# spaceandtimefdn/blitzar

Hardware: AMD Instinct MI355X
Metric: MSM throughput (scalar-point ops/sec) (higher is better)
Workload: dtype u32; 1 GPU; curve25519_msm_n2^20_252bit; columns_per_gpu=1, rows=1048576, parallelism=columns x1

## Files before the change

### __graft_entry__.py

```python
import os
import subprocess
import sys

ROOT = os.path.dirname(os.path.abspath(__file__))
if ROOT not in sys.path:
    sys.path.insert(0, ROOT)


def build():
    from blitzar_amd import build as bz_build
    bz_build.build()
    hooks_dir = os.path.join(ROOT, "tests", "native", "_build")
    os.makedirs(hooks_dir, exist_ok=True)
    hooks = os.path.join(hooks_dir, "libbz_hooks.so")
    src = os.path.join(ROOT, "tests", "native", "hooks.cpp")
    if not os.path.exists(hooks) or os.path.getmtime(hooks) < os.path.getmtime(src):
        subprocess.run(["g++", "-O2", "-std=c++20", "-fPIC", "-shared", "-I" + ROOT, src, "-o", hooks],
                       check=True)
    src = os.path.join(ROOT, "tests", "native", "tile_digest_check.cc")
    newest = max(os.path.getmtime(src),
                 os.path.getmtime(os.path.join(ROOT, "blitzar_amd", "csrc", "msm", "tile_digest.h")))
    for exe, flags in (("tile_digest_check", ["-O2"]),
                       ("tile_digest_check_san", ["-O1", "-g", "-fsanitize=address,undefined",
                                                  "-fno-sanitize-recover=all"])):
        exe = os.path.join(hooks_dir, exe)
        if not os.path.exists(exe) or os.path.getmtime(exe) < newest:
            subprocess.run(["g++", *flags, "-std=c++20", "-I" + ROOT, src, "-o", exe], check=True)
    pb_dir = os.path.join(ROOT, "tools", "pipeline_bench")
    lib_so = os.path.join(ROOT, "blitzar_amd", "lib", "libblitzar_amd.so")
    os.makedirs(os.path.join(pb_dir, "_build"), exist_ok=True)
    for tool in ("pipeline_bench", "multi_device_check", "hostapi_bench", "caller_table_bench"):
        exe = os.path.join(pb_dir, "_build", tool)
        src = os.path.join(pb_dir, tool + ".cc")
        if (not os.path.exists(exe)
                or os.path.getmtime(exe) < max(os.path.getmtime(src), os.path.getmtime(lib_so))):
            subprocess.run(["/opt/rocm/bin/hipcc", "-O2", "-std=c++17",
                            "-I" + os.path.join(ROOT, "include"), "-I" + pb_dir, src,
                            "-L" + os.path.dirname(lib_so), "-lblitzar_amd",
                            "-Wl,-rpath,$ORIGIN/../../../blitzar_amd/lib", "-o", exe], check=True)
    mc_src = os.path.join(ROOT, "tools", "multi_commitment", "benchmark.cc")
    mc_exe = os.path.join(ROOT, "tools", "multi_commitment", "_build", "multi_commitment")
    os.makedirs(os.path.dirname(mc_exe), exist_ok=True)
    if (not os.path.exists(mc_exe)
            or os.path.getmtime(mc_exe) < max(os.path.getmtime(mc_src), os.path.getmtime(lib_so))):
        subprocess.run(["g++", "-O2", "-std=c++17", "-I" + os.path.join(ROOT, "include"), mc_src,
                        "-L" + os.path.dirname(lib_so), "-lblitzar_amd",
                        "-Wl,-rpath,$ORIGIN/../../../blitzar_amd/lib", "-Wl,-rpath,/opt/rocm/lib",
                        "-o", mc_exe], check=True)
    exe = os.path.join(hooks_dir, "sig_ours")
    src = os.path.join(ROOT, "tests", "native", "boundary", "signatures.cc")
    if (not os.path.exists(exe)
            or os.path.getmtime(exe) < max(os.path.getmtime(src), os.path.getmtime(lib_so))):
        subprocess.run(["g++", "-O1", "-std=c++17", "-I" + os.path.join(ROOT, "include"),
                        '-DBZ_API_HEADER="blitzar_api.h"', src, "-L" + os.path.dirname(lib_so),
                        "-lblitzar_amd", "-Wl,-rpath,$ORIGIN/../../../blitzar_amd/lib",
                        "-Wl,-rpath,/opt/rocm/lib", "-o", exe], check=True)
    mt_dir = os.path.join(ROOT, "tools", "mt19937")
    mt_so = os.path.join(mt_dir, "_build", "libmtstream.so")
    mt_src = os.path.join(mt_dir, "mtstream.cc")
    os.makedirs(os.path.dirname(mt_so), exist_ok=True)
    if not os.path.exists(mt_so) or os.path.getmtime(mt_so) < os.path.getmtime(mt_src):
        subprocess.run(["g++", "-O2", "-std=c++17", "-fPIC", "-shared", "-pthread", mt_src, "-o",
                        mt_so], check=True)
    subprocess.run([sys.executable, os.path.join(ROOT, "oracle", "ref", "build_ref.py")], check=True)
    from tests import device_hooks
    device_hooks.build()
    import blitzar_amd.api as api
    api.load()


def smoke():
    import numpy as np
    from blitzar_amd import api
    from oracle import ref_oracle
    lib = api.load()
    assert lib.bzamd_device_count() > 0, "smoke() needs a GPU"
    api.reset_for_testing()
# ... 28 lines not shown
```

### blitzar_amd/csrc/msm/curve_traits.h

```cpp
#pragma once

#include "blitzar_amd/csrc/curve/ed25519.h"
#include "blitzar_amd/csrc/curve/ed29.h"
#include "blitzar_amd/csrc/curve/ed16_wave.h"
#include "blitzar_amd/csrc/curve/sw29.h"
#include "blitzar_amd/csrc/curve/sw29_coop.h"
#include "blitzar_amd/csrc/curve/sw_wave.h"
#include "blitzar_amd/csrc/curve/weierstrass.h"

namespace bz {

template <int N> struct sw_api_affine {
  u64 X[N];
  u64 Y[N];
  u8 infinity;
};
static_assert(sizeof(sw_api_affine<4>) == 72);
static_assert(sizeof(sw_api_affine<6>) == 104);

struct ed25519_msm {
  static constexpr unsigned curve_id = 0;
  using point = ed29_point;
  using addend = ed29_cached_packed;
  using api_projective = ed_point;
// ... 8 lines not shown
  static constexpr double call_table_entry_cost = 1.0;

  BZ_HD static point identity() { return ed29::identity(); }
  BZ_HD static point add(const point& a, const point& b) { return ed29::add(a, b); }
  BZ_HD static point dbl_n(const point& a, int k) { return ed29::dbl_n(a, k); }
  BZ_HD static point neg(const point& a) { return ed29::neg(a); }
  BZ_HD static void accumulate(point& acc, const addend& q, bool negate) {
    acc = ed29::add_cached(acc, ed29::unpack(q), negate);
  }
  using operand = ed29_cached;
  BZ_HD static operand stage(const addend& q) {
    operand o = ed29::unpack(q);
    f29::pin(o.YpX);
    f29::pin(o.YmX);
    f29::pin(o.Z);
    f29::pin(o.T2d);
    return o;
  }
  BZ_HD static void accumulate(point& acc, const operand& q, bool negate) {
    acc = ed29::add_cached(acc, q, negate);
  }
  static constexpr bool has_signed_gather = true;
  BZ_HD static addend gather(const addend* table, u32 row, bool negate) {
    return ed29::gather_signed(table, row, negate);
  }
  BZ_HD static void accumulate_gathered(point& acc, const operand& q, bool negate) {
    acc = ed29::add_cached_presigned(acc, q, negate);
  }
  static constexpr bool first_pinned = true;
  BZ_HD static point first_gathered(const operand& q, bool negate) {
    return ed29::from_cached_presigned(q, negate);
  }
  BZ_HD static addend make_addend(const void* api_generators, u64 i) {
    return ed29::pack(ed29::cached_from_ed(static_cast<const ed_point*>(api_generators)[i]));
  }
  BZ_HD static addend addend_from_api_projective(const void* projective, u64 i) {
    return make_addend(projective, i);
  }
  BZ_HD static void encode(u8* out, const point& p) { ristretto29::encode(out, p); }
  BZ_HD static void store_projective(u8* out, const point& p) {
    *reinterpret_cast<ed_point*>(out) = ed29::to_ed(p);
  }
  BZ_HD static point point_from_api_projective(const void* projective, u64 i) {
    return ed29::from_ed(static_cast<const ed_point*>(projective)[i]);
  }
  BZ_HD static void store_api_generator(u8* out, const point& p) { store_projective(out, p); }
  BZ_HD static point point_from_api_generator(const void* api_generators, u64 i) {
    return point_from_api_projective(api_generators, i);
  }
  static constexpr u32 batch_points_per_lane = 4;
  using batch_fe = fe29;
  BZ_HD static fe29 batch_one() { return f29::one(); }
  BZ_HD static fe29 batch_mul(const fe29& a, const fe29& b) { return f29::mul(a, b); }
  BZ_HD static fe29 batch_z(const point& p, bool& is_identity) {
    is_identity = false;
    return p.Z;
  }
  static constexpr size_t compact_size = 120;
  BZ_HD static void store_compact(u8* out, const point& p, const fe29& zinv, bool) {
    const fe29 x = f29::mul(p.X, zinv), y = f29::mul(p.Y, zinv);
    const fe51 c[3] = {f29::to_fe51(x), f29::to_fe51(y), f29::to_fe51(f29::mul(x, y))};
    u64* o = reinterpret_cast<u64*>(out);
    for (int k = 0; k < 3; ++k)
      for (int i = 0; i < 5; ++i) o[5 * k + i] = c[k].v[i];
  }
#if defined(__HIPCC__)
  __device__ static fe29 batch_wave_invert(const fe29& z) {
    const ed16w::lane_ctx c = ed16w::make_ctx(ed16w::wave_scratch());
    const fe29 t = ed16w::pow22523(c, z);
    return f29::mul(f29::sqn(t, 3), f29::mul(f29::sq(z), z));
  }
#endif
  static constexpr bool has_wave_horner = true;
#if defined(__HIPCC__)
  __device__ static point wave_horner(const point& acc, bool have_acc, point* window_sums,
                                      u32 stride, u32 num_windows, u32 window_bits) {
    const ed16w::lane_ctx c = ed16w::make_ctx(ed16w::wave_scratch());
    for (u32 w = c.lane; w < num_windows; w += 64) {
      point* slot = window_sums + static_cast<size_t>(w) * stride;
      const ed29_cached_packed q = ed29::pack(ed29::to_cached(*slot));
      *reinterpret_cast<ed29_cached_packed*>(slot) = q;
    }
    ed16w::wave_lds_sync();
    u32 state = ed16w::identity(c);
    if (have_acc) state = ed16w::load_point(c, acc);
    for (u32 i = num_windows; i-- > 0;) {
      if (have_acc || i + 1 != num_windows) {
        for (u32 k = 0; k < window_bits; ++k) state = ed16w::dbl(c, state);
      }
      const u32* q = reinterpret_cast<const u32*>(window_sums + static_cast<size_t>(i) * stride);
      state = ed16w::add_cached(c, state, ed16w::load_words(c, q));
    }
    return ed16w::store_point(c, state);
  }
  __device__ static void wave_chain(point* out, u64 stride, const point& g, u32 windows, u32 bits) {
    const ed16w::lane_ctx c = ed16w::make_ctx(ed16w::wave_scratch());
    u32 state = ed16w::load_point(c, g);
#pragma unroll 1
    for (u32 w = 0;; ++w) {
      const point p = ed16w::store_point(c, state);
      if (c.lane == 0) out[static_cast<u64>(w) * stride] = p;
      if (w + 1 >= windows) break;
#pragma unroll 1
      for (u32 k = 0; k < bits; ++k) state = ed16w::dbl(c, state);
    }
  }
  static constexpr bool has_wave_add_multiple = true;
  static constexpr bool reduce_scan_few_columns_only = false;
  __device__ static point wave_add_multiple(const point& v, const point& s, u32 m) {
    __shared__ ed29_cached_packed addend[2];
    const ed16w::lane_ctx c = ed16w::make_ctx(ed16w::wave_scratch());
    if (c.lane < 2) addend[c.lane] = ed29::pack(ed29::to_cached(c.lane == 0 ? s : v));
    ed16w::wave_lds_sync();
    const u32 sq = ed16w::load_words(c, addend[0].w), vq = ed16w::load_words(c, addend[1].w);
    u32 state = ed16w::identity(c);
    for (int bit = 31 - __builtin_clz(m); bit >= 0; --bit) {
      state = ed16w::dbl(c, state);
      if ((m >> bit) & 1) state = ed16w::add_cached(c, state, sq);
    }
    state = ed16w::add_cached(c, state, vq);
    return ed16w::store_point(c, state);
  }
  static constexpr bool has_wave_encode = true;
  static constexpr bool has_coop_add = false;
  __device__ static void wave_encode(u8* out, const point& p) {
    const ed16w::lane_ctx c = ed16w::make_ctx(ed16w::wave_scratch());
    u64 w[4];
    ristretto29::encode_words(w, p, [&c](const fe29& z) { return ed16w::pow22523(c, z); });
    if (c.lane == 0) {
      for (int i = 0; i < 4; ++i)
        for (int j = 0; j < 8; ++j) out[8 * i + j] = static_cast<u8>(w[i] >> (8 * j));
    }
  }
#endif
};

struct ed25519_niels_msm : ed25519_msm {
  using addend = ed29_niels;
  static constexpr int accumulate_launch_waves = accumulate_waves_per_simd;
  BZ_HD static void accumulate(point& acc, const addend& q, bool negate) {
    acc = ed29::add_niels(acc, q, negate);
  }
  BZ_HD static point first(const addend& q, bool negate) { return ed29::from_niels(q, negate); }
  static constexpr bool has_signed_gather = false;
  static constexpr double call_table_entry_cost = 0.88;
  using operand = ed29_niels;
  BZ_HD static operand stage(const addend& q) {
    operand o = q;
    f29::pin(o.YpX);
    f29::pin(o.YmX);
    f29::pin(o.T2d);
    return o;
  }
  BZ_HD static addend make_addend(const void* api_generators, u64 i) {
    return ed29::to_niels(ed29::from_ed(static_cast<const ed_point*>(api_generators)[i]));
  }
  BZ_HD static addend addend_from_api_projective(const void* projective, u64 i) {
    return make_addend(projective, i);
  }
  static constexpr bool has_batched_prepare = true;
  BZ_HD static fe29 batch_load_z(const void* api_generators, u64 i) {
    return f29::from_fe51(static_cast<const ed_point*>(api_generators)[i].Z);
  }
  BZ_HD static addend batch_make_addend(const void* api_generators, u64 i, const fe29& zinv) {
    const ed_point& g = static_cast<const ed_point*>(api_generators)[i];
    return niels_of(f29::from_fe51(g.X), f29::from_fe51(g.Y), zinv);
  }
  BZ_HD static addend addend_from_point(const point& p, const fe29& zinv, bool) {
    return niels_of(p.X, p.Y, zinv);
  }
  BZ_HD static addend niels_of(const fe29& big_x, const fe29& big_y, const fe29& zinv) {
    const fe29 x = f29::mul(big_x, zinv);
    const fe29 y = f29::mul(big_y, zinv);
    ed29_niels n;
    n.YpX = f29::weak_reduce(f29::add(y, x));
    n.YmX = f29::weak_reduce(f29::sub(y, x));
    n.T2d = f29::mul(f29::mul(x, y), f29::const_2d());
    for (int k = 0; k < 5; ++k) n.pad[k] = 0;
    return n;
  }
};

template <class G29, unsigned CurveId> struct sw_msm_base {
  static constexpr unsigned curve_id = CurveId;
  static constexpr double call_table_entry_cost = 1.0;
  using G64 = typename G29::G64;
  using F64 = typename G64::F;
  static constexpr int N64 = F64::N;
  using point = typename G29::point;
  using addend = typename G29::packed;
  using api_projective = typename G64::point;
  using api_affine = sw_api_affine<N64>;
  static constexpr size_t api_generator_size = sizeof(api_affine);
  static constexpr size_t projective_size = sizeof(api_projective);
  static constexpr int accumulate_waves_per_simd = G29::N <= 9 ? 3 : 2;
  static constexpr int accumulate_launch_waves = accumulate_waves_per_simd;
  static constexpr bool accumulate_pinned = G29::N <= 9;
  static constexpr bool has_batched_prepare = false;
  static constexpr bool has_signed_gather = false;
  static constexpr bool has_wave_encode = false;
  static constexpr bool has_wave_add_multiple = true;
  static constexpr bool reduce_scan_few_columns_only = true;
#if defined(__HIPCC__)
  __device__ static point wave_add_multiple(const point& v, const point& s, u32 m) {
    using W = sww::wave<G29>;
    const typename W::ctx c = W::make_ctx(sww::wave_scratch());
    const u32 sq = W::load_point_value(c, s), vq = W::load_point_value(c, v);
    u32 st = sq;
    for (int bit = 30 - __builtin_clz(m); bit >= 0; --bit) {
      st = W::dbl(c, st);
      if ((m >> bit) & 1) st = W::add(c, st, sq);
    }
    return W::store_point(c, W::add(c, st, vq));
  }
#endif
  static constexpr bool has_wave_horner = true;
// ... 149 lines not shown
```

### blitzar_amd/csrc/msm/curve_tu.h

```cpp
#pragma once

#include "blitzar_amd/csrc/msm/dispatch.h"
#include "blitzar_amd/csrc/msm/engine.h"
#include "blitzar_amd/csrc/fixed/partition_table.h"
#include "blitzar_amd/csrc/fixed/partition_table_device.h"
#include "blitzar_amd/csrc/msm/host_backend.h"

namespace bz {

template <class C>
__global__ void __launch_bounds__(256)
    k_prepare_addends_projective(typename C::addend* __restrict__ addends,
                                 const typename C::api_projective* __restrict__ points, u64 n) {
  const u64 i = static_cast<u64>(blockIdx.x) * blockDim.x + threadIdx.x;
  if (i >= n) return;
  addends[i] = C::addend_from_api_projective(points, i);
}

template <class C, bool Encode = true>
__global__ void __launch_bounds__(64)
    k_fold_encode(u8* __restrict__ out, const typename C::api_projective* __restrict__ partials,
                  u32 num_partials, u32 num_outputs) {
  const u32 k = blockIdx.x * blockDim.x + threadIdx.x;
  if (k >= num_outputs) return;
// ... 158 lines not shown
    launch_prepare_addends<R>(static_cast<typename R::addend*>(d_addends), d_api_generators, n,
                              stream);
    BZ_HIP_CHECK(hipGetLastError());
  }
  static void prepare_resident_projective(void* d_addends, const void* d_projective, u64 n,
                                          hipStream_t stream) {
    if (n == 0) return;
    hipLaunchKernelGGL((k_prepare_addends_projective<R>), dim3(ceil_div_u32(n, 256)), dim3(256), 0,
                       stream, static_cast<typename R::addend*>(d_addends),
                       static_cast<const typename R::api_projective*>(d_projective), n);
    BZ_HIP_CHECK(hipGetLastError());
  }
  static const typename R::addend* build_call_table(msm_context& ctx, const void* d_api_generators,
                                                    u64 n, const window_table& t,
                                                    hipStream_t stream) {
    using point = typename R::point;
    using addend = typename R::addend;
    const u64 rows = t.stride * t.windows;
    ctx.call_table.reset(device_arena::padded(sizeof(addend) * (rows + 1)) +
                             device_arena::padded(sizeof(point) * (rows + 1)),
                         stream);
    addend* table = ctx.call_table.take<addend>(rows + 1);
    point* points = ctx.call_table.take<point>(rows + 1);
    hipStream_t bs = stream;
    if (ctx.table_overlap) {
      ctx.make_side_stream();
      ctx.table_fork.record(stream);
      ctx.table_fork.wait(ctx.side);
      bs = ctx.side;
    }
    if (t.stride <= wave_chain_max_rows<R>() && ctx.wave_chain) {
      hipLaunchKernelGGL((k_chain_points_wave<R>), dim3(static_cast<u32>(t.stride)), dim3(64), 0, bs,
                         points, d_api_generators, n, t.stride, t.windows, t.bits);
    } else {
      hipLaunchKernelGGL((k_chain_points<R>), dim3(ceil_div_u32(t.stride, 64)), dim3(64), 0, bs,
                         points, d_api_generators, n, t.stride, t.windows, static_cast<int>(t.bits));
    }
    hipLaunchKernelGGL((k_points_to_addends<R>),
                       dim3(ceil_div_u32(rows, 256ull * R::batch_points_per_lane)), dim3(256), 0, bs,
                       table, points, rows);
    BZ_HIP_CHECK(hipGetLastError());
    g_kernel_launches += 2;
    ctx.call_tables_built += 1;
    ctx.call_table_rows = table;
    if (ctx.table_overlap) {
      ctx.table_ready.record(bs);
      ctx.table_pending = true;
    }
    return table;
  }
  static const typename R::addend* call_table_locked(msm_context& ctx,
                                                     const std::vector<host_column>& cols,
                                                     const void* d_api_generators,
                                                     window_table& shape, hipStream_t stream) {
    shape = window_table{};
    shape.windows = 0;
    if (!ctx.call_tables || d_api_generators == nullptr) return nullptr;
    const call_table_choice ch =
        choose_call_table(cols, ctx.tuning, sizeof(typename R::addend), R::call_table_entry_cost,
                          ctx.force_call_table_bits);
    if (ch.shape.windows == 0) return nullptr;
    const u64 n = generator_rows_of(cols);
    shape = ch.shape;
    return build_call_table(ctx, d_api_generators, n, shape, stream);
  }
  static const void* call_table(msm_context& ctx, const std::vector<host_column>& cols,
                                const void* d_api_generators, window_table* shape,
                                hipStream_t stream) {
    std::lock_guard<std::recursive_mutex> lock(ctx.mu);
    ctx.order_after_previous(stream);
    const void* table = call_table_locked(ctx, cols, d_api_generators, *shape, stream);
    if (table != nullptr) ctx.mark_enqueued(stream);
    return table;
  }
  static void msm(msm_context& ctx, u8* d_out, u32 out_stride, bool projective_out,
                  const std::vector<host_column>& cols, const void* d_addends,
                  const void* d_api_generators, hipStream_t stream, bool generators_keyed) {
    if (cols.empty()) return;
    std::lock_guard<std::recursive_mutex> lock(ctx.mu);
    configure_sort_kernels(ctx);
    ctx.order_after_previous(stream);
    if (d_addends == nullptr) {
      window_table shape;
      const typename R::addend* table = call_table_locked(ctx, cols, d_api_generators, shape, stream);
      if (table != nullptr) {
        msm_enqueue_locked<R>(ctx, d_out, out_stride, projective_out, cols, table, nullptr, stream,
                              &shape, ctx.force_call_table_bits != 0);
        return;
      }
    }
    msm_enqueue_locked<C>(ctx, d_out, out_stride, projective_out, cols,
                          static_cast<const typename C::addend*>(d_addends), d_api_generators, stream,
                          nullptr, false, generators_keyed);
  }
  static void prepare_addends(void* d_addends, const void* d_api_generators, u64 n,
                              hipStream_t stream) {
    launch_prepare_addends<C>(static_cast<typename C::addend*>(d_addends), d_api_generators, n,
                              stream);
    BZ_HIP_CHECK(hipGetLastError());
  }
  static void prepare_addends_projective(void* d_addends, const void* d_projective, u64 n,
                                         hipStream_t stream) {
    if (n == 0) return;
    hipLaunchKernelGGL((k_prepare_addends_projective<C>), dim3(ceil_div_u32(n, 256)), dim3(256), 0,
                       stream, static_cast<typename C::addend*>(d_addends),
                       static_cast<const typename C::api_projective*>(d_projective), n);
    BZ_HIP_CHECK(hipGetLastError());
  }
  static void msm_host_entry(u8* out, u32 out_stride, bool projective_out,
                             const std::vector<host_column>& cols, const void* generators,
                             bool generators_projective, u64 num_generators) {
    std::vector<typename H::addend> addends(num_generators);
    for (u64 i = 0; i < num_generators; ++i) {
      addends[i] = generators_projective
                       ? H::addend_from_api_projective(generators, i)
                       : H::make_addend(generators, i);
    }
    msm_host<H>(out, out_stride, projective_out, cols, addends.data());
  }
  static void fold_encode_host(u8* out, const void* partials, u32 num_partials, u32 num_outputs) {
    for (u32 k = 0; k < num_outputs; ++k) {
      typename C::point acc = C::identity();
      for (u32 r = 0; r < num_partials; ++r) {
        acc = C::add(acc,
                     C::point_from_api_projective(partials, static_cast<u64>(r) * num_outputs + k));
      }
      C::encode(out + static_cast<u64>(k) * C::output_size, acc);
    }
  }
  static void fold_shifted_host(u8* out, const void* pieces, const u32* piece_counts,
                                u32 num_outputs, u32 shift_bits) {
    u64 first = 0;
    for (u32 k = 0; k < num_outputs; ++k) {
      typename C::point acc = C::identity();
      for (u32 j = piece_counts[k]; j-- > 0;) {
        if (j + 1 != piece_counts[k]) acc = C::dbl_n(acc, static_cast<int>(shift_bits));
        acc = C::add(acc, C::point_from_api_projective(pieces, first + j));
      }
      C::store_projective(out + static_cast<u64>(k) * C::projective_size, acc);
      first += piece_counts[k];
// ... 59 lines not shown
```

### blitzar_amd/csrc/msm/engine.h

```cpp
#pragma once

#include <cstdlib>
#include <cstring>
#include <mutex>
#include <type_traits>
#include <vector>

#include "blitzar_amd/csrc/base/device.h"
#include "blitzar_amd/csrc/msm/kernels.h"

namespace bz {

constexpr int kNumStages = 6;
struct stage_timer {
  struct span {
    int stage;
    hipEvent_t begin, end;
  };
  bool enabled = false;
  std::vector<span> spans;
  size_t calls = 0;
  size_t capacity_calls = 0;

  unsigned stage_mask = 0x3f;
// ... 51 lines not shown
};

struct stage_mark {
  hipEvent_t ev = nullptr;
  hipStream_t on = nullptr;
  bool set = false;
  void record(hipStream_t stream) {
    if (ev == nullptr) BZ_HIP_CHECK(hipEventCreateWithFlags(&ev, hipEventDisableTiming));
    BZ_HIP_CHECK(hipEventRecord(ev, stream));
    on = stream;
    set = true;
  }
  void wait(hipStream_t stream) const {
    if (!set || stream == on) return;
    BZ_HIP_CHECK(hipStreamWaitEvent(stream, ev, 0));
  }
  void destroy() {
    if (ev != nullptr) (void)hipEventDestroy(ev);
    ev = nullptr;
    set = false;
  }
};

struct msm_context {
  device_arena arena;
  host_stage_ring descriptors;
  msm_tuning tuning;
  stage_timer timer;
  std::recursive_mutex mu;
  hipEvent_t last_done = nullptr;
  hipStream_t last_stream = nullptr;
  bool has_last = false;
  bool kernels_configured = false;
  hipStream_t tail = nullptr, tail2 = nullptr;
  stage_mark acc_done[4], reduce_done[4], horner_done[4];
  u64 reduce_joined = 0;
  hipStream_t reduce_joined_on = nullptr;
  device_arena call_table;
  hipStream_t side = nullptr;
  stage_mark table_fork, table_ready;
  bool table_pending = false;
  bool call_tables = true;
  bool table_overlap = true;
  bool wave_chain = true;
  u32 force_call_table_bits = 0;
  u64 call_tables_built = 0;
  const void* call_table_rows = nullptr;
  void make_side_stream() {
    if (side != nullptr) return;
    BZ_HIP_CHECK(hipStreamCreateWithFlags(&side, hipStreamNonBlocking));
  }
  struct caller_slot {
    unsigned curve = 0;
    size_t addend_size = 0;
    const void* key = nullptr;
    void* addends = nullptr;
    tile_digest* tiles = nullptr;
    tile_digest* rows = nullptr;
    size_t addend_bytes = 0;
    u64 capacity_rows = 0;
    u64 valid_rows = 0;
    u64 last_use = 0;
    void release() {
      for (void* p : {addends, static_cast<void*>(tiles), static_cast<void*>(rows)}) {
        if (p != nullptr) (void)hipFree(p);
      }
      *this = caller_slot{};
    }
  };
  caller_slot caller_slots[2];
  u64 caller_clock = 0;
  bool caller_table = true;
  static constexpr size_t kConvertedBytes =
      sizeof(unsigned long long) * kConvertedCounters * kConvertedCounterStride;
  unsigned long long* tiles_converted = nullptr;
  void release_caller_slots() {
    for (auto& s : caller_slots) s.release();
  }
  caller_slot* caller_slot_for(unsigned curve, size_t addend_size, const void* key, u64 rows,
                               hipStream_t stream) {
    caller_slot* slot = nullptr;
    for (auto& s : caller_slots) {
      if (s.key == key && s.curve == curve && s.addend_size == addend_size) slot = &s;
    }
    if (slot == nullptr) {
      slot = caller_slots[0].last_use <= caller_slots[1].last_use ? &caller_slots[0] : &caller_slots[1];
      slot->curve = curve;
      slot->addend_size = addend_size;
      slot->key = key;
      slot->valid_rows = 0;
    }
    if (tiles_converted == nullptr) {
      BZ_HIP_CHECK(hipMalloc(reinterpret_cast<void**>(&tiles_converted), kConvertedBytes));
      BZ_HIP_CHECK(hipMemsetAsync(tiles_converted, 0, kConvertedBytes, stream));
    }
    const size_t need_bytes = addend_size * (rows + 1);
    if (need_bytes > slot->addend_bytes || rows > slot->capacity_rows) {
      const caller_slot keep = *slot;
      slot->release();
      slot->curve = keep.curve;
      slot->addend_size = keep.addend_size;
      slot->key = keep.key;
      const u64 cap = rows > keep.capacity_rows ? rows : keep.capacity_rows;
      const size_t bytes = need_bytes > keep.addend_bytes ? need_bytes : keep.addend_bytes;
      if (hipMalloc(&slot->addends, bytes) != hipSuccess ||
          hipMalloc(reinterpret_cast<void**>(&slot->tiles), sizeof(tile_digest) * ((cap + 63) / 64)) !=
              hipSuccess ||
          hipMalloc(reinterpret_cast<void**>(&slot->rows), sizeof(tile_digest) * cap) != hipSuccess) {
        (void)hipGetLastError();
        slot->release();
        return nullptr;
      }
      slot->addend_bytes = bytes;
      slot->capacity_rows = cap;
    }
    slot->last_use = ++caller_clock;
    return slot;
  }
  u64 seq = 0;
  u64 joined = 0;
  hipStream_t joined_on = nullptr;
  u64 pipe_layout = 0;
  bool defer_tail = false;
  bool overlap_tails = true;
  u32 compact_reduce = 2;
  bool slow_instruction_fetch = false;
  u32 device_cus = 0;
  u32 stream_cus(hipStream_t stream) {
    if (device_cus == 0) {
      int device = 0, cus = 0;
      BZ_HIP_CHECK(hipGetDevice(&device));
      BZ_HIP_CHECK(hipDeviceGetAttribute(&cus, hipDeviceAttributeMultiprocessorCount, device));
      device_cus = cus > 0 ? static_cast<u32>(cus) : 1;
    }
    u32 usable = device_cus;
    if (stream != nullptr) {
      uint32_t mask[32] = {};
      if (hipExtStreamGetCUMask(stream, 32, mask) == hipSuccess) {
        u32 bits = 0;
        for (u32 w = 0; w < 32; ++w) bits += static_cast<u32>(__builtin_popcount(mask[w]));
        if (bits != 0 && bits < usable) usable = bits;
      } else {
        (void)hipGetLastError();
      }
    }
    return usable;
  }
  void make_pipe_streams() {
    if (tail != nullptr) return;
    int least = 0, greatest = 0;
    BZ_HIP_CHECK(hipDeviceGetStreamPriorityRange(&least, &greatest));
    BZ_HIP_CHECK(hipStreamCreateWithPriority(&tail, hipStreamNonBlocking, least));
    BZ_HIP_CHECK(hipStreamCreateWithPriority(&tail2, hipStreamNonBlocking, least));
// ... 107 lines not shown
  front += device_arena::padded(sizeof(u32) * 2 * (plan.total_buckets + 1));
  front += device_arena::padded(sizeof(u32) * (plan.total_segments + 1));
  const size_t ends = device_arena::padded(sizeof(u32) * (plan.total_buckets + 1));
  size_t tail = 0;
  tail += device_arena::padded(sizeof(point) * (plan.total_buckets + 1));
  tail += device_arena::padded(sizeof(point) * (plan.total_segments + 1));
  tail += device_arena::padded(sizeof(point) * (num_tasks * partial_stride + 1));
  tail += device_arena::padded(sizeof(point) * (num_cols + 1));
  tail += device_arena::padded(sizeof(u32) * (num_tasks + 1));
  return front + mode.end_sets() * ends + mode.tail_sets() * tail;
}

static inline u32 partial_stride_of(const msm_plan& plan) {
  return plan.max_task_buckets == 0 ? 1 : ceil_div_u32(plan.max_task_buckets, plan.reduce_block_buckets());
}

template <class C>
void msm_enqueue_batch(msm_context& ctx, u8* d_out, u32 out_stride, bool projective_out,
                       const msm_plan& plan, const typename C::addend* d_addends,
                       const void* d_api_generators, hipStream_t stream, pipe_mode mode,
                       msm_context::caller_slot* slot = nullptr);

template <class C>
void msm_enqueue_locked(msm_context& ctx, u8* d_out, u32 out_stride, bool projective_out,
                        const std::vector<host_column>& cols, const typename C::addend* d_addends,
                        const void* d_api_generators, hipStream_t stream,
                        const window_table* tables = nullptr, bool force_tables = false,
                        bool generators_keyed = false);

template <class C>
void msm_enqueue(msm_context& ctx, u8* d_out, u32 out_stride, bool projective_out,
                 const std::vector<host_column>& cols, const typename C::addend* d_addends,
                 const void* d_api_generators, hipStream_t stream,
                 const window_table* tables = nullptr) {
  if (cols.empty()) return;
  std::lock_guard<std::recursive_mutex> lock(ctx.mu);
  configure_sort_kernels(ctx);
  ctx.order_after_previous(stream);
  msm_enqueue_locked<C>(ctx, d_out, out_stride, projective_out, cols, d_addends, d_api_generators,
                        stream, tables);
}

template <class C>
void msm_enqueue_locked(msm_context& ctx, u8* d_out, u32 out_stride, bool projective_out,
                        const std::vector<host_column>& cols, const typename C::addend* d_addends,
                        const void* d_api_generators, hipStream_t stream,
                        const window_table* tables, bool force_tables, bool generators_keyed) {
  size_t nonempty_columns = 0;
  for (const auto& c : cols) nonempty_columns += c.n != 0 ? 1 : 0;
  pipe_mode mode;
  mode.piped = ctx.defer_tail && ctx.overlap_tails && nonempty_columns < ctx.tuning.defer_max_columns;
  ctx.defer_tail = false;
  msm_context::caller_slot* slot = nullptr;
  if (generators_keyed && ctx.caller_table && d_addends == nullptr && d_api_generators != nullptr &&
      caller_table_applies<C>(d_api_generators) && generator_rows_of(cols) != 0) {
    slot = ctx.caller_slot_for(C::curve_id, sizeof(typename C::addend), d_api_generators,
                               generator_rows_of(cols), stream);
  }
  if constexpr (C::has_batched_prepare) {
    BZ_RELEASE_ASSERT(d_addends != nullptr, "Z = 1 addends come from a resident generator set");
  }
  msm_tuning tune = ctx.tuning;
  tune.in_sequence = mode.piped;
  if (force_tables) tune.force_window_tables = true;
  tune.accumulate_wave_slots =
      static_cast<u32>(C::accumulate_waves_per_simd) * 4 * ctx.stream_cus(stream);
  bool any_signed = false;
  for (const auto& c : cols) any_signed = any_signed || c.is_signed;
  if (any_signed && tune.max_window_bits > 15) tune.max_window_bits = 15;
  if (tables != nullptr) {
    const double table_bytes = static_cast<double>(sizeof(typename C::addend)) *
                               static_cast<double>(tables->stride) * tables->windows;
    tune.table_penalty = table_bytes > 200.0 * (1 << 20) ? 1.15 : 1.03;
  }

  std::vector<msm_plan> batches;
  std::vector<size_t> first_column;
  size_t need = 0;
  const bool needs_addends = d_addends == nullptr && slot == nullptr;
  auto plan_range = [&](size_t begin, size_t end, size_t& bytes) {
    msm_plan p = make_msm_plan(std::vector<host_column>(cols.begin() + begin, cols.begin() + end),
                               tune, tables);
    bytes = msm_workspace_bytes<C>(p, needs_addends, partial_stride_of(p), mode);
    return p;
  };
  auto fits = [&](const msm_plan& p, size_t bytes) {
    return p.tasks.size() <= tune.max_tasks_per_batch && p.columns.size() <= 32768 &&
           bytes <= tune.max_workspace_bytes;
  };
  for (size_t begin = 0; begin < cols.size();) {
    size_t bytes = 0;
    size_t end = cols.size();
    msm_plan plan = plan_range(begin, end, bytes);
    if (!fits(plan, bytes) && end - begin > 1) {
      size_t lo = begin + 1, hi = end;
      {
        const double by_tasks = static_cast<double>(tune.max_tasks_per_batch) /
                                static_cast<double>(plan.tasks.size() ? plan.tasks.size() : 1);
        const double by_bytes = static_cast<double>(tune.max_workspace_bytes) /
                                static_cast<double>(bytes ? bytes : 1);
        const double share = 0.97 * (by_tasks < by_bytes ? by_tasks : by_bytes);
        const size_t guess = begin + static_cast<size_t>(static_cast<double>(end - begin) * share);
        if (guess > begin + 1 && guess < end) {
          size_t guess_bytes = 0;
          msm_plan p = plan_range(begin, guess, guess_bytes);
          if (fits(p, guess_bytes)) {
            if (guess_bytes > need) need = guess_bytes;
            first_column.push_back(begin);
            batches.push_back(std::move(p));
            begin = guess;
            continue;
          }
          hi = guess;
// ... 370 lines not shown
```

### blitzar_amd/csrc/msm/kernels.h

```cpp
#pragma once

#include <utility>

#include "blitzar_amd/csrc/msm/curve_traits.h"
#include "blitzar_amd/csrc/msm/plan.h"
#include "blitzar_amd/csrc/msm/recode.h"
#include "blitzar_amd/csrc/msm/tile_digest.h"

namespace bz {

using i16 = int16_t;
using i32 = int32_t;
template <class D> inline constexpr u32 kDigitsPerVector = 16 / sizeof(D);

constexpr u32 kSortThreads = 1024;
constexpr u32 kReduceHeavyHeads = 16;
constexpr u32 kReduceMaxHeavy = 8;
constexpr u32 kAccumulateThreads = 256;
constexpr u32 kCombineThreads = 256;

template <class C>
__global__ void __launch_bounds__(256)
    k_prepare_addends(typename C::addend* __restrict__ addends, const void* __restrict__ api_generators,
                      u64 n) {
  const u64 i = static_cast<u64>(blockIdx.x) * blockDim.x + threadIdx.x;
  if (i >= n) return;
  addends[i] = C::make_addend(api_generators, i);
}

__device__ __forceinline__ void wave_lds_fence() {
  __builtin_amdgcn_fence(__ATOMIC_RELEASE, "workgroup");
  __builtin_amdgcn_wave_barrier();
  __builtin_amdgcn_fence(__ATOMIC_ACQUIRE, "workgroup");
}
struct caller_table_view {
  tile_digest* tiles;
  tile_digest* rows;
  u64 valid_rows;
  unsigned long long* converted;
};
constexpr u32 kConvertedCounters = 256, kConvertedCounterStride = 16;
template <class C, bool Table = false>
__global__ void __launch_bounds__(256)
    k_prepare_addends_staged(typename C::addend* __restrict__ addends,
                             const void* __restrict__ api_generators, u64 n,
                             caller_table_view table) {
  using addend = typename C::addend;
  constexpr u32 G = static_cast<u32>(C::api_generator_size);
  constexpr u32 A = static_cast<u32>(sizeof(addend));
  static_assert(G % 8 == 0 && A % 16 == 0 && A <= G && (64 * G) % 16 == 0);
  __shared__ __attribute__((aligned(16))) u8 stage[4 * 64 * G];
  const u32 lane = threadIdx.x & 63;
  const u32 wave = Table ? __builtin_amdgcn_readfirstlane(threadIdx.x >> 6) : threadIdx.x >> 6;
  const u64 first = (static_cast<u64>(blockIdx.x) * 4 + wave) * 64;
  if (first >= n) return;
  const u32 count = static_cast<u32>(n - first < 64 ? n - first : 64);
  u8* region = stage + wave * (64 * G);
  const u8* src = static_cast<const u8*>(api_generators) + first * G;
  const u32 in_bytes = count * G;
  const u64 tile = first >> 6;
  tile_digest state{}, stored{};
  bool tile_known = false;
  if constexpr (Table) {
    tile_known = first < table.valid_rows;
    if (tile_known) stored = table.tiles[tile];
    state = digest_lane_begin(lane, count);
  }
  constexpr u32 kRounds = (64 * G / 16 + 63) / 64;
  uint4 words[kRounds];
#pragma unroll
  for (u32 r = 0; r < kRounds; ++r) {
    const u32 off = (r * 64 + lane) * 16;
    if (off + 16 <= in_bytes) words[r] = *reinterpret_cast<const uint4*>(src + off);
  }
#pragma unroll
  for (u32 r = 0; r < kRounds; ++r) {
    const u32 off = (r * 64 + lane) * 16;
    if (off + 16 <= in_bytes) {
      const uint4 v = words[r];
      *reinterpret_cast<uint4*>(region + off) = v;
      if constexpr (Table) {
        state = digest_absorb(state, off >> 4, v.x | static_cast<u64>(v.y) << 32,
                              v.z | static_cast<u64>(v.w) << 32);
      }
    }
  }
  if ((in_bytes & 8) != 0 && lane == 0) {
    const u64 v = *reinterpret_cast<const u64*>(src + in_bytes - 8);
    *reinterpret_cast<u64*>(region + in_bytes - 8) = v;
    if constexpr (Table) state = digest_absorb(state, in_bytes >> 4, v, 0);
  }
  tile_digest whole{}, mine{};
  if constexpr (Table) {
    state = digest_lane_end(state);
    for (int m = 32; m >= 1; m >>= 1) {
      state.a ^= __shfl_xor(state.a, m, 64);
      state.b ^= __shfl_xor(state.b, m, 64);
    }
    whole = digest_finish(state, count);
    if (tile_known && stored.a == whole.a && stored.b == whole.b) return;
  }
  wave_lds_fence();
  if constexpr (Table) {
    const bool known = lane < count && first + lane < table.valid_rows;
    tile_digest was{};
    if (known) was = table.rows[first + lane];
    bool same = lane >= count;
    if (lane < count) {
      mine = digest_of_row(reinterpret_cast<const u64*>(region + lane * G), G, lane);
      same = known && was.a == mine.a && was.b == mine.b;
    }
    if (__all(same)) {
      if (count == 64 && lane == 0) table.tiles[tile] = whole;
      return;
    }
  }
  addend a;
  if (lane < count) a = C::make_addend(region, lane);
  wave_lds_fence();
  if (lane < count) *reinterpret_cast<addend*>(region + lane * A) = a;
  wave_lds_fence();
  u8* dst = reinterpret_cast<u8*>(addends + first);
  const u32 out_bytes = count * A;
  for (u32 off = lane * 16; off < out_bytes; off += 64 * 16) {
    *reinterpret_cast<uint4*>(dst + off) = *reinterpret_cast<const uint4*>(region + off);
  }
  if constexpr (Table) {
    if (lane < count) table.rows[first + lane] = mine;
    if (lane == 0) {
      table.tiles[tile] = whole;
      atomicAdd(table.converted + (tile % kConvertedCounters) * kConvertedCounterStride, 1ull);
    }
  }
}

constexpr u32 kBatchPrepareThreads = 256;
constexpr u32 kBatchPreparePoints = 4;
template <u32 N, class F> __device__ __forceinline__ void static_for(F&& f) {
  [&]<u32... J>(std::integer_sequence<u32, J...>) {
    (f(std::integral_constant<u32, J>{}), ...);
  }(std::make_integer_sequence<u32, N>{});
}
template <class C, u32 T>
__device__ __forceinline__ void tree_products(typename C::batch_fe* tree, u32 tid) {
  __syncthreads();
  for (u32 s = T / 2; s >= 1; s >>= 1) {
    if (tid < s) tree[s + tid] = C::batch_mul(tree[2 * (s + tid)], tree[2 * (s + tid) + 1]);
    __syncthreads();
  }
}
template <class C, u32 T>
__device__ __forceinline__ void tree_inverses(typename C::batch_fe* tree, u32 tid) {
  __syncthreads();
  for (u32 s = 1; s < T; s <<= 1) {
    if (tid < s) {
      const u32 i = s + tid;
      const typename C::batch_fe inv = tree[i], left = tree[2 * i], right = tree[2 * i + 1];
      tree[2 * i] = C::batch_mul(inv, right);
      tree[2 * i + 1] = C::batch_mul(inv, left);
    }
    __syncthreads();
  }
}

template <class C>
__global__ void __launch_bounds__(kBatchPrepareThreads, 1)
    k_prepare_addends_batched(typename C::addend* __restrict__ addends,
                              const void* __restrict__ api_generators, u64 n) {
  using fe = typename C::batch_fe;
  __shared__ fe tree[2 * kBatchPrepareThreads];
  const u32 tid = threadIdx.x;
  const u64 base = static_cast<u64>(blockIdx.x) * kBatchPrepareThreads * kBatchPreparePoints;
  fe z[kBatchPreparePoints], prefix[kBatchPreparePoints];
  static_for<kBatchPreparePoints>([&](auto jc) {
    constexpr u32 j = decltype(jc)::value;
    const u64 i = base + static_cast<u64>(j) * kBatchPrepareThreads + tid;
    z[j] = i < n ? C::batch_load_z(api_generators, i) : C::batch_one();
    if constexpr (j == 0) {
      prefix[0] = z[0];
    } else {
      prefix[j] = C::batch_mul(prefix[j - 1], z[j]);
    }
  });
  tree[kBatchPrepareThreads + tid] = prefix[kBatchPreparePoints - 1];
  tree_products<C, kBatchPrepareThreads>(tree, tid);
  if (tid < 64) {
    const fe inv = C::batch_wave_invert(tree[1]);
    if (tid == 0) tree[1] = inv;
  }
  tree_inverses<C, kBatchPrepareThreads>(tree, tid);
  fe inv = tree[kBatchPrepareThreads + tid];
  static_for<kBatchPreparePoints>([&](auto jc) {
    constexpr u32 j = kBatchPreparePoints - 1 - decltype(jc)::value;
    fe zinv = inv;
    if constexpr (j != 0) {
      zinv = C::batch_mul(inv, prefix[j - 1]);
      inv = C::batch_mul(inv, z[j]);
    }
    const u64 i = base + static_cast<u64>(j) * kBatchPrepareThreads + tid;
    if (i < n) addends[i] = C::batch_make_addend(api_generators, i, zinv);
  });
}

template <class C>
void launch_prepare_addends(typename C::addend* d_addends, const void* d_api_generators, u64 n,
                            hipStream_t stream) {
  if (n == 0) return;
  if constexpr (C::has_batched_prepare) {
    const u64 per_block = static_cast<u64>(kBatchPrepareThreads) * kBatchPreparePoints;
    hipLaunchKernelGGL((k_prepare_addends_batched<C>), dim3(ceil_div_u32(n, per_block)),
                       dim3(kBatchPrepareThreads), 0, stream, d_addends, d_api_generators, n);
  } else if ((reinterpret_cast<uintptr_t>(d_api_generators) & 15) == 0 &&
             (reinterpret_cast<uintptr_t>(d_addends) & 15) == 0) {
    hipLaunchKernelGGL((k_prepare_addends_staged<C, false>), dim3(ceil_div_u32(n, 256)), dim3(256),
                       0, stream, d_addends, d_api_generators, n, caller_table_view{});
  } else {
    hipLaunchKernelGGL((k_prepare_addends<C>), dim3(ceil_div_u32(n, 256)), dim3(256), 0, stream,
                       d_addends, d_api_generators, n);
  }
}

template <class C> bool caller_table_applies(const void* d_api_generators) {
  return !C::has_batched_prepare && (reinterpret_cast<uintptr_t>(d_api_generators) & 15) == 0;
}
template <class C>
void launch_prepare_addends_tabled(typename C::addend* d_addends, const void* d_api_generators,
                                   u64 n, const caller_table_view& table, hipStream_t stream) {
  if (n == 0) return;
  hipLaunchKernelGGL((k_prepare_addends_staged<C, true>), dim3(ceil_div_u32(n, 256)), dim3(256), 0,
                     stream, d_addends, d_api_generators, n, table);
}

template <class D>
__global__ void __launch_bounds__(256)
    k_recode(D* __restrict__ digits, const column_desc* __restrict__ columns,
             const task_desc* __restrict__ tasks, u32 num_columns, u32 num_chunks,
             u32* __restrict__ zero, u64 zero_words) {
  for (u64 i = static_cast<u64>(blockIdx.x) * blockDim.x + threadIdx.x; i < zero_words;
       i += static_cast<u64>(gridDim.x) * blockDim.x) {
    zero[i] = 0;
  }
  const u64 chunk_groups = (num_chunks + 7) / 8;
  const u64 total = 8 * chunk_groups * num_columns;
  for (u64 id = blockIdx.x; id < total; id += gridDim.x) {
    const u32 xcd = static_cast<u32>(id & 7);
    const u64 rest = id >> 3;
    const column_desc col = columns[rest % num_columns];
    const u64 chunk = (rest / num_columns) * 8 + xcd;
    const u64 row = chunk * blockDim.x + threadIdx.x;
    if (col.merged_stride != 0) {
      if (row >= col.merged_stride) continue;
      D* dst = digits + tasks[col.first_task].entry_base + row;
      digit_recoder rec;
      if (row < col.n) {
        rec.init(col.data + row * col.row_stride, col.bit_offset, col.bit_width, false,
                 col.window_bits);
      }
      for (u32 wi = 0; wi < col.num_windows; ++wi) {
        const int d = row < col.n ? rec.next() : 0;
        if (wi + 1 < col.num_windows || row < col.n) {
          dst[static_cast<u64>(wi) * col.merged_stride] = static_cast<D>(-d);
        }
      }
      continue;
    }
    if (row >= col.n) continue;
    digit_recoder rec;
    rec.init(col.data + row * col.row_stride, col.bit_offset, col.bit_width, col.is_signed != 0,
             col.window_bits);
    for (u32 wi = 0; wi < col.num_windows; ++wi) {
      const int d = rec.next();
      digits[tasks[col.first_task + wi].entry_base + row] = static_cast<D>(-d);
    }
  }
}

// ... 1471 lines not shown
```

Before: 1.156 billion scalar-point ops/s.

## Cache Z-normalised addends in caller table via batched inversion in staged kernel

Extends the caller-table prepare kernel so curves with batched prepare can build Z=1 (normalised) addends in place, using a block-wide product tree and one wave inversion per block. The caller slot is keyed by whether its entries are normalised. The call-table cost model treats the plain resident form as cost 1.0, and when no call table is chosen the MSM runs from the caller's generators through the resident-form path. The aim is to give non-resident generator calls the cheaper affine-style addends and to skip reconversion of unchanged tiles, at the cost of extra block-wide syncs and a tree inversion inside the staged kernel.

```diff
diff --git a/__graft_entry__.py b/__graft_entry__.py
--- a/__graft_entry__.py
+++ b/__graft_entry__.py
@@ -23,6 +23,16 @@
     for exe, flags in (("tile_digest_check", ["-O2"]),
                        ("tile_digest_check_san", ["-O1", "-g", "-fsanitize=address,undefined",
                                                   "-fno-sanitize-recover=all"])):
+        exe = os.path.join(hooks_dir, exe)
+        if not os.path.exists(exe) or os.path.getmtime(exe) < newest:
+            subprocess.run(["g++", *flags, "-std=c++20", "-I" + ROOT, src, "-o", exe], check=True)
+    src = os.path.join(ROOT, "tests", "native", "batch_normalise_check.cc")
+    newest = os.path.getmtime(src)
+    for d, _, fs in os.walk(os.path.join(ROOT, "blitzar_amd", "csrc")):
+        newest = max([newest] + [os.path.getmtime(os.path.join(d, f)) for f in fs if f.endswith(".h")])
+    for exe, flags in (("batch_normalise_check", ["-O2"]),
+                       ("batch_normalise_check_san", ["-O1", "-g", "-fsanitize=address,undefined",
+                                                      "-fno-sanitize-recover=all"])):
         exe = os.path.join(hooks_dir, exe)
         if not os.path.exists(exe) or os.path.getmtime(exe) < newest:
             subprocess.run(["g++", *flags, "-std=c++20", "-I" + ROOT, src, "-o", exe], check=True)
diff --git a/blitzar_amd/csrc/msm/batch_tree.h b/blitzar_amd/csrc/msm/batch_tree.h
--- /dev/null
+++ b/blitzar_amd/csrc/msm/batch_tree.h
@@ -0,0 +1,24 @@
+#pragma once
+
+#include "blitzar_amd/csrc/base/macros.h"
+
+namespace bz {
+
+template <class C>
+BZ_HD void tree_product_step(typename C::batch_fe* tree, u32 s, u32 tid) {
+  if (tid < s) tree[s + tid] = C::batch_mul(tree[2 * (s + tid)], tree[2 * (s + tid) + 1]);
+}
+template <class C>
+BZ_HD void tree_inverse_step(typename C::batch_fe* tree, u32 s, u32 tid) {
+  if (tid < s) {
+    const u32 i = s + tid;
+    const typename C::batch_fe inv = tree[i], left = tree[2 * i], right = tree[2 * i + 1];
+    tree[2 * i] = C::batch_mul(inv, right);
+    tree[2 * i + 1] = C::batch_mul(inv, left);
+  }
+}
+template <class C>
+BZ_HD typename C::batch_fe tree_leaf(const typename C::batch_fe& z, bool live) {
+  return live && !C::batch_is_zero(z) ? z : C::batch_one();
+}
+}
diff --git a/blitzar_amd/csrc/msm/curve_traits.h b/blitzar_amd/csrc/msm/curve_traits.h
--- a/blitzar_amd/csrc/msm/curve_traits.h
+++ b/blitzar_amd/csrc/msm/curve_traits.h
@@ -84,6 +84,7 @@
   using batch_fe = fe29;
   BZ_HD static fe29 batch_one() { return f29::one(); }
   BZ_HD static fe29 batch_mul(const fe29& a, const fe29& b) { return f29::mul(a, b); }
+  BZ_HD static bool batch_is_zero(const fe29& a) { return f29::is_zero(a); }
   BZ_HD static fe29 batch_z(const point& p, bool& is_identity) {
     is_identity = false;
     return p.Z;
@@ -98,7 +99,10 @@
   }
 #if defined(__HIPCC__)
   __device__ static fe29 batch_wave_invert(const fe29& z) {
-    const ed16w::lane_ctx c = ed16w::make_ctx(ed16w::wave_scratch());
+    return batch_wave_invert(z, ed16w::wave_scratch());
+  }
+  __device__ static fe29 batch_wave_invert(const fe29& z, ed16w::scratch* lds) {
+    const ed16w::lane_ctx c = ed16w::make_ctx(lds);
     const fe29 t = ed16w::pow22523(c, z);
     return f29::mul(f29::sqn(t, 3), f29::mul(f29::sq(z), z));
   }
@@ -194,6 +198,16 @@
   BZ_HD static fe29 batch_load_z(const void* api_generators, u64 i) {
     return f29::from_fe51(static_cast<const ed_point*>(api_generators)[i].Z);
   }
+  BZ_HD static void batch_load_xyz(const void* api_generators, u64 i, fe29& big_x, fe29& big_y,
+                                   fe29& z) {
+    const ed_point& g = static_cast<const ed_point*>(api_generators)[i];
+    big_x = f29::from_fe51(g.X);
+    big_y = f29::from_fe51(g.Y);
+    z = f29::from_fe51(g.Z);
+  }
+#if defined(__HIPCC__)
+  using batch_scratch = ed16w::scratch;
+#endif
   BZ_HD static addend batch_make_addend(const void* api_generators, u64 i, const fe29& zinv) {
     const ed_point& g = static_cast<const ed_point*>(api_generators)[i];
     return niels_of(f29::from_fe51(g.X), f29::from_fe51(g.Y), zinv);
diff --git a/blitzar_amd/csrc/msm/curve_tu.h b/blitzar_amd/csrc/msm/curve_tu.h
--- a/blitzar_amd/csrc/msm/curve_tu.h
+++ b/blitzar_amd/csrc/msm/curve_tu.h
@@ -234,12 +234,14 @@
   static const typename R::addend* call_table_locked(msm_context& ctx,
                                                      const std::vector<host_column>& cols,
                                                      const void* d_api_generators,
-                                                     window_table& shape, hipStream_t stream) {
+                                                     window_table& shape, hipStream_t stream,
+                                                     bool plain_is_resident_form = false) {
     shape = window_table{};
     shape.windows = 0;
     if (!ctx.call_tables || d_api_generators == nullptr) return nullptr;
     const call_table_choice ch =
-        choose_call_table(cols, ctx.tuning, sizeof(typename R::addend), R::call_table_entry_cost,
+        choose_call_table(cols, ctx.tuning, sizeof(typename R::addend),
+                          plain_is_resident_form ? 1.0 : R::call_table_entry_cost,
                           ctx.force_call_table_bits);
     if (ch.shape.windows == 0) return nullptr;
     const u64 n = generator_rows_of(cols);
@@ -263,11 +265,21 @@
     configure_sort_kernels(ctx);
     ctx.order_after_previous(stream);
     if (d_addends == nullptr) {
+      const bool resident_form = !std::is_same_v<C, R> && generators_keyed && ctx.caller_table &&
+                                 d_api_generators != nullptr &&
+                                 caller_table_applies<R>(d_api_generators) &&
+                                 generator_rows_of(cols) != 0;
       window_table shape;
-      const typename R::addend* table = call_table_locked(ctx, cols, d_api_generators, shape, stream);
+      const typename R::addend* table =
+          call_table_locked(ctx, cols, d_api_generators, shape, stream, resident_form);
       if (table != nullptr) {
         msm_enqueue_locked<R>(ctx, d_out, out_stride, projective_out, cols, table, nullptr, stream,
                               &shape, ctx.force_call_table_bits != 0);
+        return;
+      }
+      if (resident_form) {
+        msm_enqueue_locked<R>(ctx, d_out, out_stride, projective_out, cols, nullptr, d_api_generators,
+                              stream, nullptr, false, true);
         return;
       }
     }
diff --git a/blitzar_amd/csrc/msm/engine.h b/blitzar_amd/csrc/msm/engine.h
--- a/blitzar_amd/csrc/msm/engine.h
+++ b/blitzar_amd/csrc/msm/engine.h
@@ -127,6 +127,7 @@
   }
   struct caller_slot {
     unsigned curve = 0;
+    bool normalised = false;
     size_t addend_size = 0;
     const void* key = nullptr;
     void* addends = nullptr;
@@ -152,15 +153,19 @@
   void release_caller_slots() {
     for (auto& s : caller_slots) s.release();
   }
-  caller_slot* caller_slot_for(unsigned curve, size_t addend_size, const void* key, u64 rows,
-                               hipStream_t stream) {
+  caller_slot* caller_slot_for(unsigned curve, bool normalised, size_t addend_size, const void* key,
+                               u64 rows, hipStream_t stream) {
     caller_slot* slot = nullptr;
     for (auto& s : caller_slots) {
-      if (s.key == key && s.curve == curve && s.addend_size == addend_size) slot = &s;
+      if (s.key == key && s.curve == curve && s.normalised == normalised &&
+          s.addend_size == addend_size) {
+        slot = &s;
+      }
     }
     if (slot == nullptr) {
       slot = caller_slots[0].last_use <= caller_slots[1].last_use ? &caller_slots[0] : &caller_slots[1];
       slot->curve = curve;
+      slot->normalised = normalised;
       slot->addend_size = addend_size;
       slot->key = key;
       slot->valid_rows = 0;
@@ -174,6 +179,7 @@
       const caller_slot keep = *slot;
       slot->release();
       slot->curve = keep.curve;
+      slot->normalised = keep.normalised;
       slot->addend_size = keep.addend_size;
       slot->key = keep.key;
       const u64 cap = rows > keep.capacity_rows ? rows : keep.capacity_rows;
@@ -387,13 +393,17 @@
   mode.piped = ctx.defer_tail && ctx.overlap_tails && nonempty_columns < ctx.tuning.defer_max_columns;
   ctx.defer_tail = false;
   msm_context::caller_slot* slot = nullptr;
-  if (generators_keyed && ctx.caller_table && d_addends == nullptr && d_api_generators != nullptr &&
-      caller_table_applies<C>(d_api_generators) && generator_rows_of(cols) != 0) {
-    slot = ctx.caller_slot_for(C::curve_id, sizeof(typename C::addend), d_api_generators,
-                               generator_rows_of(cols), stream);
+  const bool caller_table_offered = generators_keyed && ctx.caller_table && d_addends == nullptr &&
+                                    d_api_generators != nullptr &&
+                                    caller_table_applies<C>(d_api_generators) &&
+                                    generator_rows_of(cols) != 0;
+  if (caller_table_offered) {
+    slot = ctx.caller_slot_for(C::curve_id, C::has_batched_prepare, sizeof(typename C::addend),
+                               d_api_generators, generator_rows_of(cols), stream);
   }
   if constexpr (C::has_batched_prepare) {
-    BZ_RELEASE_ASSERT(d_addends != nullptr, "Z = 1 addends come from a resident generator set");
+    BZ_RELEASE_ASSERT(d_addends != nullptr || caller_table_offered,
+                      "Z = 1 addends come from a resident generator set or the context's caller table");
   }
   msm_tuning tune = ctx.tuning;
   tune.in_sequence = mode.piped;
diff --git a/blitzar_amd/csrc/msm/kernels.h b/blitzar_amd/csrc/msm/kernels.h
--- a/blitzar_amd/csrc/msm/kernels.h
+++ b/blitzar_amd/csrc/msm/kernels.h
@@ -2,6 +2,7 @@
 
 #include <utility>
 
+#include "blitzar_amd/csrc/msm/batch_tree.h"
 #include "blitzar_amd/csrc/msm/curve_traits.h"
 #include "blitzar_amd/csrc/msm/plan.h"
 #include "blitzar_amd/csrc/msm/recode.h"
@@ -26,6 +27,23 @@
   const u64 i = static_cast<u64>(blockIdx.x) * blockDim.x + threadIdx.x;
   if (i >= n) return;
   addends[i] = C::make_addend(api_generators, i);
+}
+
+template <class C, u32 T>
+__device__ __forceinline__ void tree_products(typename C::batch_fe* tree, u32 tid) {
+  __syncthreads();
+  for (u32 s = T / 2; s >= 1; s >>= 1) {
+    tree_product_step<C>(tree, s, tid);
+    __syncthreads();
+  }
+}
+template <class C, u32 T>
+__device__ __forceinline__ void tree_inverses(typename C::batch_fe* tree, u32 tid) {
+  __syncthreads();
+  for (u32 s = 1; s < T; s <<= 1) {
+    tree_inverse_step<C>(tree, s, tid);
+    __syncthreads();
+  }
 }
 
 __device__ __forceinline__ void wave_lds_fence() {
@@ -46,6 +64,8 @@
                              const void* __restrict__ api_generators, u64 n,
                              caller_table_view table) {
   using addend = typename C::addend;
+  constexpr bool Norm = Table && C::has_batched_prepare;
+  static_assert(Table || !C::has_batched_prepare, "Z = 1 addends outside a table: the batched kernel");
   constexpr u32 G = static_cast<u32>(C::api_generator_size);
   constexpr u32 A = static_cast<u32>(sizeof(addend));
   static_assert(G % 8 == 0 && A % 16 == 0 && A <= G && (64 * G) % 16 == 0);
@@ -53,8 +73,11 @@
   const u32 lane = threadIdx.x & 63;
   const u32 wave = Table ? __builtin_amdgcn_readfirstlane(threadIdx.x >> 6) : threadIdx.x >> 6;
   const u64 first = (static_cast<u64>(blockIdx.x) * 4 + wave) * 64;
-  if (first >= n) return;
-  const u32 count = static_cast<u32>(n - first < 64 ? n - first : 64);
+  if constexpr (!Norm) {
+    if (first >= n) return;
+  }
+  const u32 count = first >= n ? 0 : static_cast<u32>(n - first < 64 ? n - first : 64);
+  bool convert = count != 0;
   u8* region = stage + wave * (64 * G);
   const u8* src = static_cast<const u8*>(api_generators) + first * G;
   const u32 in_bytes = count * G;
@@ -62,7 +85,7 @@
   tile_digest state{}, stored{};
   bool tile_known = false;
   if constexpr (Table) {
-    tile_known = first < table.valid_rows;
+    tile_known = convert && first < table.valid_rows;
     if (tile_known) stored = table.tiles[tile];
     state = digest_lane_begin(lane, count);
   }
@@ -98,10 +121,13 @@
       state.b ^= __shfl_xor(state.b, m, 64);
     }
     whole = digest_finish(state, count);
-    if (tile_known && stored.a == whole.a && stored.b == whole.b) return;
-  }
-  wave_lds_fence();
-  if constexpr (Table) {
+    if (tile_known && stored.a == whole.a && stored.b == whole.b) {
+      if constexpr (!Norm) return;
+      convert = false;
+    }
+  }
+  if (convert) wave_lds_fence();
+  if (Table && convert) {
     const bool known = lane < count && first + lane < table.valid_rows;
     tile_digest was{};
     if (known) was = table.rows[first + lane];
@@ -112,12 +138,45 @@
     }
     if (__all(same)) {
       if (count == 64 && lane == 0) table.tiles[tile] = whole;
-      return;
+      if constexpr (!Norm) return;
+      convert = false;
     }
   }
   addend a;
-  if (lane < count) a = C::make_addend(region, lane);
-  wave_lds_fence();
+  if constexpr (Norm) {
+    using fe = typename C::batch_fe;
+    constexpr u32 T = 256;
+    static_assert(sizeof(fe) * 2 * T % 16 == 0 &&
+                  sizeof(fe) * 2 * T + sizeof(typename C::batch_scratch) <= sizeof(stage));
+    const bool live = convert && lane < count;
+    fe big_x, big_y, z;
+    if (live) C::batch_load_xyz(region, lane, big_x, big_y, z);
+    wave_lds_fence();
+    if (lane == 0) *reinterpret_cast<u32*>(region) = convert ? 1u : 0u;
+    __syncthreads();
+    u32 any = 0;
+#pragma unroll
+    for (u32 w = 0; w < 4; ++w) any |= *reinterpret_cast<const u32*>(stage + w * (64 * G));
+    if (any == 0) return;
+    __syncthreads();
+    fe* tree = reinterpret_cast<fe*>(stage);
+    auto* scratch = reinterpret_cast<typename C::batch_scratch*>(stage + sizeof(fe) * 2 * T);
+    const u32 tid = threadIdx.x;
+    tree[T + tid] = live ? tree_leaf<C>(z, true) : C::batch_one();
+    tree_products<C, T>(tree, tid);
+    if (tid < 64) {
+      const fe inv = C::batch_wave_invert(tree[1], scratch);
+      if (tid == 0) tree[1] = inv;
+    }
+    tree_inverses<C, T>(tree, tid);
+    const fe zinv = tree[T + tid];
+    __syncthreads();
+    if (!convert) return;
+    if (live) a = C::niels_of(big_x, big_y, zinv);
+  } else {
+    if (lane < count) a = C::make_addend(region, lane);
+    wave_lds_fence();
+  }
   if (lane < count) *reinterpret_cast<addend*>(region + lane * A) = a;
   wave_lds_fence();
   u8* dst = reinterpret_cast<u8*>(addends + first);
@@ -141,28 +200,6 @@
     (f(std::integral_constant<u32, J>{}), ...);
   }(std::make_integer_sequence<u32, N>{});
 }
-template <class C, u32 T>
-__device__ __forceinline__ void tree_products(typename C::batch_fe* tree, u32 tid) {
-  __syncthreads();
-  for (u32 s = T / 2; s >= 1; s >>= 1) {
-    if (tid < s) tree[s + tid] = C::batch_mul(tree[2 * (s + tid)], tree[2 * (s + tid) + 1]);
-    __syncthreads();
-  }
-}
-template <class C, u32 T>
-__device__ __forceinline__ void tree_inverses(typename C::batch_fe* tree, u32 tid) {
-  __syncthreads();
-  for (u32 s = 1; s < T; s <<= 1) {
-    if (tid < s) {
-      const u32 i = s + tid;
-      const typename C::batch_fe inv = tree[i], left = tree[2 * i], right = tree[2 * i + 1];
-      tree[2 * i] = C::batch_mul(inv, right);
-      tree[2 * i + 1] = C::batch_mul(inv, left);
-    }
-    __syncthreads();
-  }
-}
-
 template <class C>
 __global__ void __launch_bounds__(kBatchPrepareThreads, 1)
     k_prepare_addends_batched(typename C::addend* __restrict__ addends,
@@ -221,7 +258,7 @@
 }
 
 template <class C> bool caller_table_applies(const void* d_api_generators) {
-  return !C::has_batched_prepare && (reinterpret_cast<uintptr_t>(d_api_generators) & 15) == 0;
+  return (reinterpret_cast<uintptr_t>(d_api_generators) & 15) == 0;
 }
 template <class C>
 void launch_prepare_addends_tabled(typename C::addend* d_addends, const void* d_api_generators,
```

Measured after the change: 1.219 billion scalar-point ops/s (median of 6 runs). +5.4%, better.
